# BUBLET/uav-airvision

Hardware: AMD Instinct MI355X
Metric: stereo frames/sec (LK+stereo+MSCKF-update) at 752x480 (higher is better)
Workload: dtype u8/int32 windows, f32 normal equations

## Files before the change

uav_airvision_amd/csrc/msckf.hip:

```cpp
#include <math.h>

#include <new>
#include <vector>

#include "av_common.h"

namespace {

constexpr int IMU_DIM = 21;

#ifndef AV_FILTER_WAVE_PRIO
#define AV_FILTER_WAVE_PRIO 3
#endif
#define AV_FILTER_PRIO() __builtin_amdgcn_s_setprio(AV_FILTER_WAVE_PRIO)

__device__ __forceinline__ double av_rsqrt_f64(double d)
{
    const bool tiny = d < 1e-280;
    const double ds = tiny ? d * 0x1p200 : d;
    double y = __builtin_amdgcn_rsq(ds);
    const double h = 0.5 * ds;
    y = y * (1.5 - h * y * y);
    y = y * (1.5 - h * y * y);
    return tiny ? y * 0x1p100 : y;
// ... 702 lines not shown
__global__ __attribute__((amdgpu_waves_per_eu(2, 3))) __launch_bounds__(256) void feature_kernel8(FeatArgs a) { feature_body<8>(a); }

static int msckf_lds_opt_in();

static int launch_feature_kernel(FeatArgs a, int cnt, int Mx, hipStream_t st)
{
    int rc0 = msckf_lds_opt_in();
    if (rc0) return rc0;
    a.Mmax = Mx; a.n_list = cnt;
    const int team = Mx <= 2 ? 16 : (Mx <= 4 ? 64 : 256);
    const size_t per = (feature_lds_bytes(Mx, team) + 7) / 8 * 8;
    a.team_doubles = (int)(per / 8);
    const size_t lds = per * (256 / team);
    if (lds > 160 * 1024) { av_set_error("MSCKF feature blocks: %d observations per feature need %zu B of LDS", Mx, lds); return AV_E_CAPACITY; }
    if (team == 16) hipLaunchKernelGGL(feature_kernel<16>, dim3((cnt + 15) / 16), dim3(256), lds, st, a);
    else if (team == 64) hipLaunchKernelGGL(feature_kernel<64>, dim3((cnt + 3) / 4), dim3(256), lds, st, a);
    else hipLaunchKernelGGL(feature_kernel<256>, dim3(cnt), dim3(256), lds, st, a);
    AV_LAUNCH_CHECK();
    return AV_OK;
}

struct PropArgs {
    double* P; int n, ld;
    double dt;
    double gyro[3], acc[3];
    double q_old[4];
    double q_new[4];
    double q_null[4], v_null[3], p_null[3];
    double v_new[3], p_new[3];
    double gravity[3];
    double noise[4];
};

constexpr int PROP_LDS_DOUBLES = 5 * IMU_DIM * IMU_DIM + IMU_DIM * 12;
template <bool EXT = false, int NT = 256>
__device__ __forceinline__ void propagate_body(const PropArgs& a, double* P11s = nullptr, double* PhiT = nullptr, double* ext = nullptr)
{
    __shared__ double own[EXT ? 1 : PROP_LDS_DOUBLES];
    double* const base = EXT ? ext : own;
    double* const F = base, * const F2 = F + IMU_DIM * IMU_DIM, * const Phi = F2 + IMU_DIM * IMU_DIM, * const T = Phi + IMU_DIM * IMU_DIM,
          * const Q = T + IMU_DIM * IMU_DIM, * const G = Q + IMU_DIM * IMU_DIM;
    __shared__ double Rwi[9], Rnull[9], Rnew[9], u[3], sv[3], w1[3], w2[3];
    const int tid = threadIdx.x;
    const int N = IMU_DIM;
    constexpr int Q1 = NT == 256 ? 64 : 1, Q2 = NT == 256 ? 128 : 2;
    constexpr int R1 = NT == 256 ? 64 : 9, R2 = NT == 256 ? 128 : 22, R3 = NT == 256 ? 192 : 43;
    for (int i = tid; i < N * N; i += NT) F[i] = 0.0;
    for (int i = tid; i < N * 12; i += NT) G[i] = 0.0;
    if (tid == 0 || tid == Q1 || tid == Q2) quat_to_rot(tid == 0 ? a.q_old : (tid == Q1 ? a.q_null : a.q_new), tid == 0 ? Rwi : (tid == Q1 ? Rnull : Rnew));
    __syncthreads();
    if (tid < 9) {
        const int r = tid / 3, c = tid - 3 * r;
        const double* w = a.gyro; const double* ac = a.acc;
        const double skw[9] = {0, -w[2], w[1], w[2], 0, -w[0], -w[1], w[0], 0};
        const double ska[9] = {0, -ac[2], ac[1], ac[2], 0, -ac[0], -ac[1], ac[0], 0};
        F[r * N + c] = -skw[r * 3 + c];
        F[r * N + 3 + c] = r == c ? -1.0 : 0.0;
        double s = 0;
        for (int k = 0; k < 3; ++k) s += Rwi[k * 3 + r] * ska[k * 3 + c];
        F[(6 + r) * N + c] = -s;
        F[(6 + r) * N + 9 + c] = -Rwi[c * 3 + r];
        F[(12 + r) * N + 6 + c] = r == c ? 1.0 : 0.0;
        G[r * 12 + c] = r == c ? -1.0 : 0.0;
        G[(3 + r) * 12 + 3 + c] = r == c ? 1.0 : 0.0;
        G[(6 + r) * 12 + 6 + c] = -Rwi[c * 3 + r];
        G[(9 + r) * 12 + 9 + c] = r == c ? 1.0 : 0.0;
    } else if (tid == R1) {
        for (int r = 0; r < 3; ++r) u[r] = Rnull[r * 3] * a.gravity[0] + Rnull[r * 3 + 1] * a.gravity[1] + Rnull[r * 3 + 2] * a.gravity[2];
        double uu = u[0] * u[0] + u[1] * u[1] + u[2] * u[2];
        for (int r = 0; r < 3; ++r) sv[r] = u[r] / uu;
    } else if (tid == R2) {
        double dv[3] = {a.v_null[0] - a.v_new[0], a.v_null[1] - a.v_new[1], a.v_null[2] - a.v_new[2]};
        double dp[3] = {a.dt * a.v_null[0] + a.p_null[0] - a.p_new[0], a.dt * a.v_null[1] + a.p_null[1] - a.p_new[1], a.dt * a.v_null[2] + a.p_null[2] - a.p_new[2]};
        const double* g = a.gravity;
        w1[0] = -dv[2] * g[1] + dv[1] * g[2]; w1[1] = dv[2] * g[0] - dv[0] * g[2]; w1[2] = -dv[1] * g[0] + dv[0] * g[1];
        w2[0] = -dp[2] * g[1] + dp[1] * g[2]; w2[1] = dp[2] * g[0] - dp[0] * g[2]; w2[2] = -dp[1] * g[0] + dp[0] * g[1];
    }
    __syncthreads();
    __shared__ unsigned frow[IMU_DIM], fcol[IMU_DIM], prow[IMU_DIM];
    for (int i = tid; i < N * N; i += NT) F[i] *= a.dt;
    if (tid >= R2 && tid < R2 + N) {
        const int r = tid - R2; unsigned m = 0;
        for (int k = 0; k < N; ++k) if (F[r * N + k] != 0.0) m |= 1u << k;
        frow[r] = m;
    } else if (tid >= R3 && tid < R3 + N) {
        const int c = tid - R3; unsigned m = 0;
        for (int k = 0; k < N; ++k) if (F[k * N + c] != 0.0) m |= 1u << k;
        fcol[c] = m;
    }
    __syncthreads();
    for (int i = tid; i < N * N; i += NT) {
        int r = i / N, c = i - r * N; double s = 0;
        for (unsigned m = frow[r]; m; m &= m - 1) { const int k = __builtin_ctz(m); s += F[r * N + k] * F[k * N + c]; }
        F2[i] = s;
    }
    __syncthreads();
    for (int i = tid; i < N * N; i += NT) {
        int r = i / N, c = i - r * N; double s = 0;
        for (unsigned m = fcol[c]; m; m &= m - 1) { const int k = __builtin_ctz(m); s += F2[r * N + k] * F[k * N + c]; }
        Phi[i] = (r == c ? 1.0 : 0.0) + F[i] + F2[i] / 2. + s / 6.;
    }
    __syncthreads();
    if (tid < 9) {
        int r = tid / 3, c = tid % 3; double s = 0;
        for (int k = 0; k < 3; ++k) s += Rnew[r * 3 + k] * Rnull[c * 3 + k];
        Phi[r * N + c] = s;
    } else if (tid >= R1 && tid < R1 + 6) {
        const int t6 = tid - R1, blk = t6 / 3, r = t6 % 3;
        const int row = (blk == 0 ? 6 : 12) + r;
        const double* wv = blk == 0 ? w1 : w2;
        const double p0 = Phi[row * N], p1 = Phi[row * N + 1], p2 = Phi[row * N + 2];
        const double Au = p0 * u[0] + p1 * u[1] + p2 * u[2];
        const double d = Au - wv[r];
        Phi[row * N] = p0 - d * sv[0]; Phi[row * N + 1] = p1 - d * sv[1]; Phi[row * N + 2] = p2 - d * sv[2];
    } else if (tid >= R2 && tid < R2 + N) {
        const int r = tid - R2; unsigned m = 0;
        for (int k = 0; k < N; ++k) if (Phi[r * N + k] != 0.0) m |= 1u << k;
        if (r < 3 || (r >= 6 && r < 9) || (r >= 12 && r < 15)) m |= 7u;
        prow[r] = m;
    }
    __syncthreads();
    for (int i = tid; i < N * 12; i += NT) {
        int r = i / 12, c = i - r * 12; double s = 0;
        for (unsigned m = prow[r]; m; m &= m - 1) { const int k = __builtin_ctz(m); s += Phi[r * N + k] * G[k * 12 + c]; }
        T[i] = s;
    }
    for (int i = tid; i < N * N; i += NT) {
        int r = i / N, c = i - r * N; double s = 0;
        if (P11s) { for (unsigned m = prow[r]; m; m &= m - 1) { const int k = __builtin_ctz(m); s += Phi[r * N + k] * P11s[k * N + c]; } }
        else      { for (unsigned m = prow[r]; m; m &= m - 1) { const int k = __builtin_ctz(m); s += Phi[r * N + k] * a.P[(size_t)k * a.ld + c]; } }
        F2[i] = s;
        if (P11s) {
            double s2 = 0;
            for (unsigned m = prow[r]; m; m &= m - 1) { const int k = __builtin_ctz(m); s2 += Phi[r * N + k] * PhiT[k * N + c]; }
            Q[i] = s2;
        }
    }
    __syncthreads();
    for (int i = tid; i < N * N; i += NT) {
        int r = i / N, c = i - r * N; double s = 0, q = 0;
        for (int k = 0; k < 12; ++k) q += T[r * 12 + k] * a.noise[k / 3] * T[c * 12 + k];
        q = q * a.dt;
        for (unsigned m = prow[c]; m; m &= m - 1) { const int k = __builtin_ctz(m); s += F2[r * N + k] * Phi[c * N + k]; }
        F[i] = s + q;
    }
    __syncthreads();
    if (P11s) {
        for (int i = tid; i < N * N; i += NT) {
            int r = i / N, c = i - r * N;
            PhiT[i] = Q[i];
            P11s[i] = (F[r * N + c] + F[c * N + r]) / 2.;
        }
        __syncthreads();
        return;
    }
    const int nc = a.n - N;
    for (int c0 = 0; c0 < nc; c0 += N) {
        const int w = min(N, nc - c0);
        for (int i = tid; i < N * w; i += NT) {
            int r = i / w, c = i - r * w; double s = 0;
            for (unsigned m = prow[r]; m; m &= m - 1) { const int k = __builtin_ctz(m); s += Phi[r * N + k] * a.P[(size_t)k * a.ld + N + c0 + c]; }
            T[i] = s;
        }
        __syncthreads();
        for (int i = tid; i < N * w; i += NT) {
            int r = i / w, c = i - r * w;
            a.P[(size_t)r * a.ld + N + c0 + c] = T[i];
            a.P[(size_t)(N + c0 + c) * a.ld + r] = T[i];
        }
        __syncthreads();
    }
    for (int i = tid; i < N * N; i += NT) {
        int r = i / N, c = i - r * N;
        a.P[(size_t)r * a.ld + c] = (F[r * N + c] + F[c * N + r]) / 2.;
    }
}

__global__ __launch_bounds__(256) void propagate_kernel(PropArgs a) { propagate_body(a); }
__global__ __launch_bounds__(256) void propagate_batch_kernel(const PropArgs* arr, const int* first)
{
    AV_FILTER_PRIO();
    __shared__ double P11s[IMU_DIM * IMU_DIM], PhiT[IMU_DIM * IMU_DIM];
    const int i0 = first[blockIdx.x], i1 = first[blockIdx.x + 1];
    if (i0 >= i1) return;
    const int tid = threadIdx.x, N = IMU_DIM;
    double* P = arr[i0].P; const int n = arr[i0].n, ld = arr[i0].ld;
    for (int i = tid; i < N * N; i += 256) { int r = i / N, c = i - r * N; P11s[i] = P[(size_t)r * ld + c]; PhiT[i] = r == c ? 1.0 : 0.0; }
    __syncthreads();
    for (int i = i0; i < i1; ++i) propagate_body(arr[i], P11s, PhiT);
    const int nc = n - N, tot = N * nc;
    constexpr int PER = (IMU_DIM * 6 * 31 + 255) / 256;
    double acc[PER];
#pragma unroll
    for (int u = 0; u < PER; ++u) {
        const int e = tid + 256 * u;
        double s = 0;
        if (e < tot) {
            const int r = e / nc, c = e - r * nc;
            for (int k = 0; k < N; ++k) s += PhiT[r * N + k] * P[(size_t)k * ld + N + c];
        }
        acc[u] = s;
// ... 1293 lines not shown
```

uav_airvision_amd/csrc/msckf_dev.inc:

```

namespace {

constexpr int DEV_BUCKETS = 2;
constexpr int DEV_IMU_BATCH = 16;
constexpr int DEV_LDS_KEYS = 2048;

enum { DFAIL_NONE = 0, DFAIL_CAMS = 1, DFAIL_FRAMES = 2, DFAIL_STACK = 3, DFAIL_PIVOT = 4, DFAIL_TABLE = 5, DFAIL_OBS = 6, DFAIL_ROWS = 7 };

struct DState {
    double ts;
    double q[4], p[3], v[3], bg[3], ba[3];
    double R_ic[9], t_ci[3];
    double qn[4], pn[3], vn[3];
    double gravity[3];
    double tracking_rate;
    long long next_imu_id;
    int n, ncam;
    int active;
    int failed;
    int first_img, null_aliased;
    int prune, rm0, rm1;
    int n_prune_steps;
    int n_two_pass;
    int resets;
};
struct DCtl {
    double t_frame;
    double q0[4], bg0[3], g0[3];
    int active, has_init, imu_first, imu_cnt;
};
struct DImu { double t, w[3], a[3]; };
struct DCov { int act, cnt, first, pad; AugArgs aa; };

struct DevArgs {
    int S, cap, FS, cs, max_cam, ld, rows_cap, obs_stride;
    unsigned long long* prof;
    int pool_rows;
    size_t pstride;
    double* P; double* scratch;
    DState* st; long long* cam_id; double* cam_q; double* cam_p; double* cam_qn; int* ncam; int* nstate; double* grav;
    int mcap, ns, hcells;
    long long* fr_id; double* fr_z; int* fr_fslot; int* fr_prev; int* fr_next; int* fr_n; int* pos_of; int* order; int* hdr; long long* births;
    long long* m_id; long long* m_birth; double* m_pos; int* m_init; int* m_nobs; int* m_tail; int* free_stack;
    int* hash_a; int* hash_b; int* hash_c; int* tmp_a; int* tmp_b; int* tmp_c; unsigned long long* keys; int* cand; int* e0; int* e1;
    int* f_off; int* obs_cam; double* obs_z; double* f_pos; int* f_dof; int* f_rowoff; int* f_valid; int* f_mslot; int* n_cand; int* over;
    int* t_off; int* t_obs_cam; double* t_obs_z;
    int* blist; int* tlist; int* cnt; int* cnt_next;
    const int* stacked; const double* dx;
    const DCtl* ctl; const DImu* imu; const long long* msg_ids; const double* msg_uv; const int* msg_n; int msg_cap;
    PropArgs* prop; DCov* cov;
    double* out;
    double R01[9], t01[3], noise[4], cov0[5];
    double trans_thr, pos_std_thr;
    double huber, precision, damping; int outer_max, inner_max;
    double* Hblk; double* rblk; size_t hstride, rstride; const double* chi2; double obs_noise; double* gamma; int* pass;
    const UpdArgs* updbase; UpdArgs* upd; int* cols; int cols_stride; int* blk_row; int* blk_len; int* stacked_out; double* work;
};

__device__ __forceinline__ TriArgs dev_tri_args(const DevArgs& a, bool prune)
{
    TriArgs t;
    t.n_feat = 0; t.obs_off = prune ? a.t_off : a.f_off; t.obs_cam = prune ? a.t_obs_cam : a.obs_cam; t.obs_z = prune ? a.t_obs_z : a.obs_z;
    t.cam_q = a.cam_q; t.cam_p = a.cam_p; t.feat_stream = nullptr; t.cam_stride = a.cs;
    for (int i = 0; i < 9; ++i) t.R01[i] = a.R01[i];
    for (int i = 0; i < 3; ++i) t.t01[i] = a.t01[i];
    t.huber = a.huber; t.precision = a.precision; t.damping = a.damping; t.outer_max = a.outer_max; t.inner_max = a.inner_max;
    t.out_pos = a.f_pos; t.out_valid = a.f_valid; t.list = nullptr; t.n_list_dev = nullptr; t.fs_stride = a.FS;
    t.f_mslot = prune ? a.f_mslot : nullptr; t.meta_pos = prune ? a.m_pos : nullptr; t.meta_init = prune ? a.m_init : nullptr; t.meta_stride = a.mcap;
    return t;
}
__device__ __forceinline__ void dev_triangulate_own(const DevArgs& a, const AvsStore& V, int s, int nc, bool prune)
{
    const TriArgs t = dev_tri_args(a, prune);
    const int wave = threadIdx.x >> 6, lane = threadIdx.x & 63;
    const size_t f0 = (size_t)s * a.FS;
    for (int k = wave; k < nc; k += (int)(blockDim.x >> 6)) if (V.tmp_b[k] >= 0) triangulate_one(t, (int)(f0 + k), lane);
    __syncthreads();
}

__device__ __forceinline__ AvsStore dev_store(const DevArgs& a, int s)
{
    AvsStore V;
    V.cap = a.cap; V.mcap = a.mcap; V.ns = a.ns; V.hcells = a.hcells;
// ... 111 lines not shown
            const int n = D->n, ld = a.ld;
            for (int k = 0; k < C.imu_cnt; ++k) {
                PropArgs pa;
                const DImu m = a.imu[C.imu_first + k];
                pa.P = P; pa.n = n; pa.ld = ld; pa.dt = m.t - D->ts;
                for (int i = 0; i < 3; ++i) { pa.gyro[i] = m.w[i] - D->bg[i]; pa.acc[i] = m.a[i] - D->ba[i]; pa.gravity[i] = D->gravity[i]; }
                for (int i = 0; i < 4; ++i) { pa.q_old[i] = D->q[i]; pa.noise[i] = a.noise[i]; }
                dev_predict_new_state(*D, pa.dt, pa.gyro, pa.acc);
                for (int i = 0; i < 4; ++i) { pa.q_new[i] = D->q[i]; pa.q_null[i] = D->qn[i]; }
                for (int i = 0; i < 3; ++i) { pa.v_null[i] = D->vn[i]; pa.p_null[i] = D->pn[i]; pa.v_new[i] = D->v[i]; pa.p_new[i] = D->p[i]; }
                for (int i = 0; i < 4; ++i) D->qn[i] = D->q[i];
                for (int i = 0; i < 3; ++i) { D->pn[i] = D->p[i]; D->vn[i] = D->v[i]; }
                D->null_aliased = 1;
                D->ts = m.t;
                a.prop[C.imu_first + k] = pa;
            }
            double Rwi[9], Rwc[9], tw[3], cq[4];
            h_to_rotation(D->q, Rwi);
            for (int r = 0; r < 3; ++r) for (int c = 0; c < 3; ++c) Rwc[r * 3 + c] = D->R_ic[r * 3] * Rwi[c] + D->R_ic[r * 3 + 1] * Rwi[3 + c] + D->R_ic[r * 3 + 2] * Rwi[6 + c];
            h_mtv(Rwi, D->t_ci, tw);
            h_to_quaternion(Rwc, cq);
            const size_t c = (size_t)s * a.cs + D->ncam;
            a.cam_id[c] = D->next_imu_id++;
            for (int i = 0; i < 4; ++i) { a.cam_q[4 * c + i] = cq[i]; a.cam_qn[4 * c + i] = cq[i]; }
            for (int i = 0; i < 3; ++i) a.cam_p[3 * c + i] = D->p[i] + tw[i];
            cv.act = 1; cv.cnt = C.imu_cnt;
            cv.aa.P = P; cv.aa.n = n; cv.aa.ld = ld;
            for (int i = 0; i < 9; ++i) cv.aa.R_ic[i] = D->R_ic[i];
            const double sk[9] = {0, -tw[2], tw[1], tw[2], 0, -tw[0], -tw[1], tw[0], 0};
            for (int i = 0; i < 9; ++i) cv.aa.sk[i] = sk[i];
            D->n = n + 6; D->ncam += 1;
            a.ncam[s] = D->ncam; a.nstate[s] = D->n;
            for (int i = 0; i < 3; ++i) a.grav[3 * s + i] = D->gravity[i];
        }
        a.cov[s] = cv;
        *Dg = L;
    }
}

template <int NT>
__global__ __launch_bounds__(NT) void dk_cov(DevArgs a)
{
    AV_FILTER_PRIO();
    __shared__ double P11s[IMU_DIM * IMU_DIM], PhiT[IMU_DIM * IMU_DIM], work[PROP_LDS_DOUBLES];
    const int s = blockIdx.x, tid = threadIdx.x, N = IMU_DIM;
    const DCov cv = a.cov[s];
    if (!cv.act) return;
    double* P = cv.aa.P;
    const int n = cv.aa.n, ld = cv.aa.ld;
    auto stamp = [&](int i) { if (a.prof && s == 0 && tid == 0) a.prof[i] = __builtin_amdgcn_s_memrealtime(); };
    stamp(0);
    if (cv.cnt > 0) {
        for (int i = tid; i < N * N; i += NT) { const int r = i / N, c = i - r * N; P11s[i] = P[(size_t)r * ld + c]; PhiT[i] = r == c ? 1.0 : 0.0; }
        __syncthreads();
        for (int k = 0; k < cv.cnt; ++k) propagate_body<true, NT>(a.prop[cv.first + k], P11s, PhiT, work);
        stamp(1);
        const int nc = n - N;
        constexpr int CW = 64, NRQ = NT / CW;
        const int cl = tid % CW, rq = tid / CW;
        for (int c0 = 0; c0 < nc; c0 += CW) {
            const int c = c0 + cl;
            const bool in = c < nc;
            __syncthreads();
            for (int k = rq; k < IMU_DIM; k += NRQ) work[k * CW + cl] = in ? P[(size_t)k * ld + N + c] : 0.0;
            __syncthreads();
#pragma unroll 1
            for (int r = rq; r < IMU_DIM; r += NRQ) {
                double sum = 0;
#pragma unroll 7
                for (int k = 0; k < IMU_DIM; ++k) sum += PhiT[r * N + k] * work[k * CW + cl];
                if (in) { P[(size_t)r * ld + N + c] = sum; P[(size_t)(N + c) * ld + r] = sum; }
            }
        }
        for (int i = tid; i < N * N; i += NT) { const int r = i / N, c = i - r * N; P[(size_t)r * ld + c] = P11s[i]; }
        __syncthreads();
    }
    stamp(2);
    augment_body<NT>(cv.aa);
}

__device__ void dev_build_candidates(const DevArgs& a, const AvsTeam& T, const AvsStore& V, int s, int nc, const int* cand, bool full,
                                     int i0, int i1, const int* e0, const int* e1, int ph, int* lb )
{
    const int tid = threadIdx.x;
    const size_t f0 = (size_t)s * a.FS, ob = (size_t)s * a.obs_stride;
    if (tid < 8) lb[tid] = 0;
    __syncthreads();
    int obs_run = 0, row_run = 0, tobs_run = 0;
    for (int base = 0; base < nc; base += (int)blockDim.x) {
        const int k = base + tid;
        const bool in = k < nc;
        const int fs = in ? cand[k] : 0;
        const int nall = in ? V.m_nobs[fs] : 0;
        const int nobs = full ? nall : (in ? 2 : 0);
        const int init = in ? V.m_init[fs] : 1;
        int to, tr, tt;
        const int o = obs_run + T.excl_scan(nobs, &to);
        const int r = row_run + T.excl_scan(in ? 4 * nobs - 3 : 0, &tr);
        const int t = tobs_run + T.excl_scan((!full && !init) ? nall : 0, &tt);
        if (in) {
            const size_t f = f0 + k;
            a.f_off[f] = (int)(ob + o); a.f_rowoff[f] = r; a.f_dof[f] = full ? nobs - 1 : 2; a.f_mslot[f] = fs;
            if (!full) a.t_off[f] = (int)(ob + t);
            if (full) (void)avs_collect(V, fs, a.obs_cam + ob + o, a.obs_z + 4 * (ob + o));
            else {
                a.obs_cam[ob + o] = i0; a.obs_cam[ob + o + 1] = i1;
                const double* z0 = V.fr_z + ((size_t)avs_lslot(e0[k]) * V.cap + avs_lidx(e0[k])) * 4;
// ... 209 lines not shown
            reset = m >= a.pos_std_thr;
        }
        s_reset = reset;
    }
    __syncthreads();
    if (s_reset) {
        AvsTeam T; T.red = red;
        const AvsStore V = dev_store(a, s);
        avs_clear(T, V);
        double* P = a.P + (size_t)s * a.pstride;
        for (int i = tid; i < IMU_DIM * IMU_DIM; i += (int)blockDim.x) {
            const int r = i / IMU_DIM, c = i - r * IMU_DIM;
            double v = 0.0;
            if (r == c) { const int blk[5] = {3, 6, 9, 15, 18}; for (int k = 0; k < 5; ++k) if (r >= blk[k] && r < blk[k] + 3) v = a.cov0[k]; }
            P[(size_t)r * a.ld + c] = v;
        }
        if (tid == 0) { D->ncam = 0; D->n = IMU_DIM; D->resets += 1; a.ncam[s] = 0; a.nstate[s] = IMU_DIM; }
    }
}
__global__ __launch_bounds__(256, 5) void dk_finish(DevArgs a)
{
    AV_FILTER_PRIO();
    dk_finish_body(a, blockIdx.x);
}


}

constexpr int DEV_RING = 3;
struct DevSlot {
    DCtl* ctl_h = nullptr; DCtl* ctl_d = nullptr;
    DImu* imu_h = nullptr; DImu* imu_d = nullptr; size_t imu_cap = 0;
    PropArgs* prop_d = nullptr;
    long long* ids_h = nullptr; double* uv_h = nullptr; int* n_h = nullptr;
    long long* ids_d = nullptr; double* uv_d = nullptr; int* n_d = nullptr;
    double* out_h = nullptr; int* cnt_h = nullptr;
    hipEvent_t done = nullptr;
    hipEvent_t t0[2] = {nullptr, nullptr}, t1[2] = {nullptr, nullptr}; bool t_used[2] = {false, false};
    bool in_flight = false;
};
struct DevPath {
    int cap = 0;
    DevArgs A;
    DevSlot slot[DEV_RING];
    double* out_d = nullptr; int* stacked0 = nullptr; int* stacked1 = nullptr; UpdArgs* updbase = nullptr; UpdArgs* upd = nullptr;
    DCov* cov_d = nullptr;
    int dk_wg = 0;
    int* cols = nullptr; int* blk_row = nullptr; int* blk_len = nullptr; int* clist = nullptr; int* again = nullptr;
    double* work = nullptr; double* gamma = nullptr; int* pass = nullptr;
    std::vector<void*> dev_allocs, host_allocs;
    int hint[16] = {0};
    bool have_hint = false;
    long long growths = 0, steps = 0;
};
```

uav_airvision_amd/csrc/msckf_dev_host.inc:

```
namespace {

constexpr int DEV_KCH = 136;

template <typename T>
int dev_alloc(DevPath* d, T** p, size_t count, int fill = 0)
{
    void* q = nullptr;
    AV_HIP(hipMalloc(&q, count * sizeof(T) + 256));
    AV_HIP(hipMemset(q, fill, count * sizeof(T) + 256));
    AV_HIP(hipStreamSynchronize(nullptr));
    d->dev_allocs.push_back(q);
    *p = reinterpret_cast<T*>(q);
    return AV_OK;
}
template <typename T>
int dev_pinned(DevPath* d, T** p, size_t count)
{
    void* q = nullptr;
    AV_HIP(hipHostMalloc(&q, count * sizeof(T) + 64, hipHostMallocDefault));
    memset(q, 0, count * sizeof(T) + 64);
    d->host_allocs.push_back(q);
    *p = reinterpret_cast<T*>(q);
    return AV_OK;
}

void dev_release(DevPath* d)
{
    if (!d) return;
    for (int k = 0; k < DEV_RING; ++k) {
        if (d->slot[k].done) (void)hipEventDestroy(d->slot[k].done);
        for (int ph = 0; ph < 2; ++ph) { if (d->slot[k].t0[ph]) (void)hipEventDestroy(d->slot[k].t0[ph]); if (d->slot[k].t1[ph]) (void)hipEventDestroy(d->slot[k].t1[ph]); }
    }
    for (void* p : d->dev_allocs) (void)hipFree(p);
    for (void* p : d->host_allocs) (void)hipHostFree(p);
    delete d;
}

__global__ __launch_bounds__(256) void dk_migrate(DevArgs o, DevArgs n)
{
    const int s = blockIdx.x, tid = threadIdx.x;
    const AvsStore A = dev_store(o, s), B = dev_store(n, s);
    for (int i = tid; i < A.ns; i += 256) { B.fr_n[i] = A.fr_n[i]; B.pos_of[i] = A.pos_of[i]; B.order[i] = A.order[i]; }
    for (int i = tid; i < AVS_HDR_WORDS; i += 256) B.hdr[i] = A.hdr[i];
    if (tid == 0) *B.births = *A.births;
    for (int sl = 0; sl < A.ns; ++sl) {
        const int cnt = A.fr_n[sl];
        for (int i = tid; i < cnt; i += 256) {
            const size_t a = (size_t)sl * A.cap + i, b = (size_t)sl * B.cap + i;
            B.fr_id[b] = A.fr_id[a]; B.fr_fslot[b] = A.fr_fslot[a]; B.fr_prev[b] = A.fr_prev[a]; B.fr_next[b] = A.fr_next[a];
            for (int e = 0; e < 4; ++e) B.fr_z[4 * b + e] = A.fr_z[4 * a + e];
        }
    }
    for (int i = tid; i < A.mcap; i += 256) {
        B.m_id[i] = A.m_id[i]; B.m_birth[i] = A.m_birth[i]; B.m_init[i] = A.m_init[i]; B.m_nobs[i] = A.m_nobs[i]; B.m_tail[i] = A.m_tail[i]; B.free_stack[i] = A.free_stack[i];
        for (int e = 0; e < 3; ++e) B.m_pos[(size_t)3 * i + e] = A.m_pos[(size_t)3 * i + e];
    }
}

int dev_reserve(av_msckf_batch* b, int cap)
{
    DevPath* d = b->dev;
    if (cap <= d->cap) return AV_OK;
    if (cap >= (1 << 24)) { av_set_error("batched MSCKF: message capacity %d exceeds the store's link format", cap); return AV_E_CAPACITY; }
    const bool grow = d->cap > 0;
// ... 2 lines not shown
    const size_t S = (size_t)b->S, cs = (size_t)b->cam_slots;
    DevArgs old = d->A;
    DevArgs& A = d->A;
    { const char* e = getenv("AV_DK_WG"); const int v = e ? atoi(e) : 0; d->dk_wg = (v == 256 || v == 64) ? v : 0; }
    A.S = b->S; A.cap = cap; A.FS = cap + 1; A.cs = b->cam_slots; A.max_cam = b->max_cam; A.ld = b->ld; A.rows_cap = b->rows_cap; A.pool_rows = (int)b_pool_rows(b, b->rows_cap);
    A.obs_stride = (int)((size_t)cap * cs); A.pstride = b->pstride; A.P = b->P; A.scratch = b->scratch;
    A.mcap = 2 * cap + 64; A.ns = b->cam_slots + 1;
    int hc = 64; while (hc < 2 * cap + 16) hc *= 2;
    A.hcells = hc;
    if ((size_t)S * A.FS >= (1u << 31) || S * (size_t)A.obs_stride >= (1u << 31)) { av_set_error("batched MSCKF: %zu streams x %d features exceed the 32-bit feature index", S, cap); return AV_E_CAPACITY; }
    const size_t nf = S * (size_t)A.FS + 8, no = S * (size_t)A.obs_stride + 8, ne = S * (size_t)A.ns * cap, nm = S * (size_t)A.mcap;
#define DA(ptr, cnt) if ((rc = dev_alloc(d, &(ptr), (size_t)(cnt)))) return rc;
#define DAF(ptr, cnt, fill) if ((rc = dev_alloc(d, &(ptr), (size_t)(cnt), fill))) return rc;
    if (!grow) {
        DA(A.st, S) DA(A.cam_id, S * cs) DA(A.cam_q, S * cs * 4) DA(A.cam_p, S * cs * 3) DA(A.cam_qn, S * cs * 4) DA(A.ncam, S) DA(A.nstate, S) DA(A.grav, S * 3)
        DA(A.n_cand, S) DA(A.over, S) DA(A.cnt, 32) DA(d->out_d, S * 12) DA(d->cov_d, S) DA(d->stacked0, S) DA(d->stacked1, S) DA(d->updbase, S) DA(d->upd, S * 2)
        DA(d->cols, S * 6 * cs) DA(d->clist, S + 8) DA(d->work, S * 8)
        DAF(A.pos_of, S * A.ns, 0xFF) DAF(A.order, S * A.ns, 0xFF) DA(A.fr_n, S * A.ns) DA(A.hdr, S * AVS_HDR_WORDS) DA(A.births, S)
    }
    DA(A.fr_id, ne) DA(A.fr_z, ne * 4) DA(A.fr_fslot, ne) DA(A.fr_prev, ne) DA(A.fr_next, ne)
    DA(A.m_id, nm) DA(A.m_birth, nm) DA(A.m_pos, nm * 3) DA(A.m_init, nm) DA(A.m_nobs, nm) DA(A.m_tail, nm) DA(A.free_stack, nm)
    DA(A.hash_a, S * hc) DA(A.hash_b, S * hc) DA(A.hash_c, S * hc)
    DA(A.tmp_a, S * cap) DA(A.tmp_b, S * cap) DA(A.tmp_c, S * cap) DA(A.keys, S * cap) DA(A.cand, S * cap) DA(A.e0, S * cap) DA(A.e1, S * cap)
    DA(A.f_off, nf) DA(A.obs_cam, no) DA(A.obs_z, no * 4) DA(A.f_pos, nf * 3) DA(A.f_dof, nf) DA(A.f_rowoff, nf) DA(A.f_valid, nf) DA(A.f_mslot, nf)
    DA(A.t_off, nf) DA(A.t_obs_cam, no) DA(A.t_obs_z, no * 4)
    DA(A.blist, 5 * S * cap + 8) DA(A.tlist, S * cap + 8) DA(d->blk_row, nf) DA(d->blk_len, nf) DA(d->again, nf) DA(d->gamma, nf) DA(d->pass, nf)
    for (int k = 0; k < DEV_RING; ++k) {
        DevSlot& sl = d->slot[k];
        if (!grow) {
            if ((rc = dev_pinned(d, &sl.ctl_h, S)) || (rc = dev_pinned(d, &sl.out_h, S * 12)) || (rc = dev_pinned(d, &sl.cnt_h, 16))) return rc;
            DA(sl.ctl_d, S) DA(sl.n_d, S)
            if ((rc = dev_pinned(d, &sl.n_h, S))) return rc;
            AV_HIP(hipEventCreateWithFlags(&sl.done, hipEventDisableTiming | hipEventBlockingSync));
            for (int ph = 0; ph < 2; ++ph) { AV_HIP(hipEventCreate(&sl.t0[ph])); AV_HIP(hipEventCreate(&sl.t1[ph])); }
        }
        DA(sl.ids_d, S * cap) DA(sl.uv_d, S * cap * 4)
        if ((rc = dev_pinned(d, &sl.ids_h, S * cap)) || (rc = dev_pinned(d, &sl.uv_h, S * cap * 4))) return rc;
    }
#undef DA
#undef DAF
    unpack_T01(b->T01, A.R01, A.t01);
    for (int i = 0; i < 4; ++i) A.noise[i] = b->noise[i];
    for (int i = 0; i < 5; ++i) A.cov0[i] = b->cov0[i];
    A.trans_thr = b->trans_thr; A.pos_std_thr = b->pos_std_thr;
    unpack_opt5(b->opt5, A);
    A.Hblk = b->Hblk; A.rblk = b->rblk; A.hstride = b->hstride; A.rstride = b->rstride; A.chi2 = b->chi2_dev; A.obs_noise = b->obs_noise;
    A.gamma = d->gamma; A.pass = d->pass; A.updbase = d->updbase; A.upd = d->upd; A.cols = d->cols; A.cols_stride = 6 * b->cam_slots;
    A.blk_row = d->blk_row; A.blk_len = d->blk_len; A.stacked_out = d->stacked1; A.work = d->work;
    A.stacked = nullptr; A.dx = b->dx; A.ctl = nullptr; A.imu = nullptr; A.prop = nullptr; A.cov = d->cov_d; A.msg_ids = nullptr; A.msg_uv = nullptr; A.msg_n = nullptr; A.msg_cap = cap; A.out = d->out_d;
    if (!grow) {
        std::vector<DState> st(S);
        for (size_t s = 0; s < S; ++s) {
            DState& D = st[s]; const BStream& T = b->st[s];
            memset(&D, 0, sizeof(D));
            D.q[3] = 1.0; D.qn[3] = 1.0; D.n = IMU_DIM; D.first_img = 1;
            for (int i = 0; i < 3; ++i) { D.v[i] = T.v[i]; D.t_ci[i] = T.t_ci[i]; D.gravity[i] = T.gravity[i]; }
            for (int i = 0; i < 9; ++i) D.R_ic[i] = T.R_ic[i];
        }
        AV_HIP(hipMemcpy(A.st, st.data(), sizeof(DState) * S, hipMemcpyHostToDevice));
        std::vector<int> n21(S, IMU_DIM);
        AV_HIP(hipMemcpy(A.nstate, n21.data(), sizeof(int) * S, hipMemcpyHostToDevice));
    } else {
        hipLaunchKernelGGL(dk_migrate, dim3((unsigned)S), dim3(256), 0, nullptr, old, A);
        AV_LAUNCH_CHECK();
        AV_HIP(hipDeviceSynchronize());
    }
    d->cap = cap;
    return AV_OK;
}

struct DevStamps {
    unsigned long long* dev = nullptr;
    int calls = 0;
    explicit DevStamps(bool on)
    {
        if (on && hipMalloc((void**)&dev, 256) == hipSuccess) { (void)hipMemset(dev, 0, 256); (void)hipStreamSynchronize(nullptr); } else dev = nullptr;
    }
    bool read(hipStream_t stm, unsigned long long t[32])
    {
        return dev && (++calls & 15) == 0 && hipStreamSynchronize(stm) == hipSuccess && hipMemcpy(t, dev, 256, hipMemcpyDeviceToHost) == hipSuccess;
    }
};
// ... 178 lines not shown
    return AV_OK;
}

int dev_enqueue(av_msckf_batch* b, int k, bool dev_msg, size_t n_imu, hipStream_t stm);

int dev_launch(av_msckf_batch* b, int k, const int64_t* ids, const double* uv, const int32_t* n_feat, int cap, const double* timestamps,
               bool dev_msg, hipEvent_t ready, hipStream_t stm)
{
    DevPath* d = b->dev;
    const int S = b->S;
    AV_HIP(hipSetDevice(b->device));
    int rc;
    if ((rc = sub_reserve(b, cap))) return rc;
    const bool first = d->cap == 0;
    const int rows_cap_before = d->A.rows_cap;
    if ((rc = dev_reserve(b, cap))) return rc;
    if (first || rows_cap_before != b->rows_cap) { if ((rc = dev_upload_updbase(b))) return rc; }
    DevSlot& sl = d->slot[k];
    if (sl.in_flight) { av_set_error("batched MSCKF: ring slot %d is still in flight", k); return AV_E_INVALID; }
    ++b->n_steps;
    if (b->debug_capture) for (BStream& T : b->st) for (int ph = 0; ph < 2; ++ph) { T.dbg_gamma[ph].clear(); T.dbg_dx[ph].clear(); T.dbg_P[ph].clear(); T.dbg_rows[ph] = 0; T.dbg_n[ph] = 0; }
    size_t n_imu = 0;
    for (int s = 0; s < S; ++s) {
        BStream& T = b->st[s];
        std::lock_guard<std::mutex> g(T.mu);
        T.active = !T.failed && T.gravity_set && timestamps[s] >= 0 && T.gravity_time <= timestamps[s];
        if (!T.active) continue;
        const double t0 = T.first_img ? timestamps[s] : T.ts;
        for (const BImu& m : T.imu) { if (m.t < t0) continue; if (m.t > timestamps[s]) break; ++n_imu; }
    }
    if (n_imu > sl.imu_cap) {
        const size_t ncap = n_imu + n_imu / 2 + (size_t)S * 16 + 64;
        if (sl.imu_cap) { AV_HIP(hipStreamSynchronize(stm)); ++d->growths; }
        if ((rc = dev_pinned(d, &sl.imu_h, ncap)) || (rc = dev_alloc(d, &sl.imu_d, ncap)) || (rc = dev_alloc(d, &sl.prop_d, ncap))) return rc;
        sl.imu_cap = ncap;
    }
    size_t w = 0;
    for (int s = 0; s < S; ++s) {
        BStream& T = b->st[s];
        DCtl& C = sl.ctl_h[s];
        C.t_frame = timestamps[s]; C.active = T.active ? 1 : 0; C.has_init = 0; C.imu_first = (int)w; C.imu_cnt = 0;
        if (!T.active) continue;
        std::lock_guard<std::mutex> g(T.mu);
        if (!T.dev_init_sent) {
            T.dev_init_sent = true; C.has_init = 1;
            for (int i = 0; i < 4; ++i) C.q0[i] = T.q[i];
            for (int i = 0; i < 3; ++i) { C.bg0[i] = T.bg[i]; C.g0[i] = T.gravity[i]; }
        }
        if (T.first_img) { T.first_img = false; T.ts = timestamps[s]; }
        size_t used = 0;
        for (const BImu& m : T.imu) {
            if (m.t < T.ts) { ++used; continue; }
            if (m.t > timestamps[s] || w >= sl.imu_cap) break;
            DImu& o = sl.imu_h[w++];
            o.t = m.t;
            for (int i = 0; i < 3; ++i) { o.w[i] = m.w[i]; o.a[i] = m.a[i]; }
            ++C.imu_cnt; ++used;
            T.ts = m.t;
        }
        T.imu.erase(T.imu.begin(), T.imu.begin() + used);
    }
    if (!dev_msg) {
        for (int s = 0; s < S; ++s) {
            const int nk = n_feat[s] < 0 ? 0 : (n_feat[s] > cap ? cap : n_feat[s]);
            sl.n_h[s] = nk;
            memcpy(sl.ids_h + (size_t)s * d->cap, ids + (size_t)s * cap, sizeof(long long) * nk);
            memcpy(sl.uv_h + (size_t)s * d->cap * 4, uv + (size_t)s * cap * 4, sizeof(double) * 4 * nk);
        }
    }
    if (dev_msg && ready) AV_HIP(hipStreamWaitEvent(stm, ready, 0));
    if ((rc = dev_enqueue(b, k, dev_msg, w, stm))) { (void)hipMemsetAsync(d->A.cnt, 0, sizeof(int) * 32, stm); return rc; }
    ++d->steps;
    AV_HIP(hipEventRecord(sl.done, stm));
    sl.in_flight = true;
    return AV_OK;
}

int dev_enqueue(av_msckf_batch* b, int k, bool dev_msg, size_t n_imu, hipStream_t stm)
{
    DevPath* d = b->dev;
    DevSlot& sl = d->slot[k];
    const int S = b->S;
    int rc;
    AV_HIP(hipMemcpyAsync(sl.ctl_d, sl.ctl_h, sizeof(DCtl) * S, hipMemcpyHostToDevice, stm));
    if (n_imu) AV_HIP(hipMemcpyAsync(sl.imu_d, sl.imu_h, sizeof(DImu) * n_imu, hipMemcpyHostToDevice, stm));
    if (!dev_msg) {
        AV_HIP(hipMemcpyAsync(sl.n_d, sl.n_h, sizeof(int) * S, hipMemcpyHostToDevice, stm));
        AV_HIP(hipMemcpyAsync(sl.ids_d, sl.ids_h, sizeof(long long) * S * d->cap, hipMemcpyHostToDevice, stm));
        AV_HIP(hipMemcpyAsync(sl.uv_d, sl.uv_h, sizeof(double) * 4 * S * d->cap, hipMemcpyHostToDevice, stm));
    }
    DevArgs a = d->A;
    a.ctl = sl.ctl_d; a.imu = sl.imu_d; a.prop = sl.prop_d; a.msg_ids = sl.ids_d; a.msg_uv = sl.uv_d; a.msg_n = sl.n_d; a.msg_cap = d->cap;
    const int par = (int)((d->steps + 1) & 1);
    a.cnt = d->A.cnt + 16 * par; a.cnt_next = d->A.cnt + 16 * (par ^ 1);
    a.prof = dev_uprof().dev ? dev_uprof().dev + 16 : nullptr;
    const int dk_wg = d->dk_wg ? d->dk_wg : (S >= 1024 ? 64 : 256);
    hipLaunchKernelGGL(dk_state, dim3((S + 63) / 64), dim3(64), 0, stm, a);
    hipLaunchKernelGGL(dk_begin4, dim3(S), dim3(dk_wg), 0, stm, a);
    if (dk_wg == 64) hipLaunchKernelGGL(dk_cov<64>, dim3(S), dim3(64), 0, stm, a);
    else hipLaunchKernelGGL(dk_cov<256>, dim3(S), dim3(256), 0, stm, a);
    AV_LAUNCH_CHECK();
    if ((rc = dev_phase(b, 0, stm, sl, a.cnt))) return rc;
    if (b->debug_capture && (rc = dev_debug_capture(b, 0, stm))) return rc;
    a.stacked = d->stacked0;
    hipLaunchKernelGGL(dk_mid, dim3(S), dim3(dk_wg), 0, stm, a);
    AV_LAUNCH_CHECK();
    if ((rc = dev_phase(b, 1, stm, sl, a.cnt))) return rc;
    if (b->debug_capture && (rc = dev_debug_capture(b, 1, stm))) return rc;
    a.stacked = d->stacked1;
    hipLaunchKernelGGL(dk_finish, dim3(S), dim3(dk_wg), 0, stm, a);
    AV_LAUNCH_CHECK();
    AV_HIP(hipMemcpyAsync(sl.out_h, d->out_d, sizeof(double) * 12 * S, hipMemcpyDeviceToHost, stm));
    AV_HIP(hipMemcpyAsync(sl.cnt_h, a.cnt, sizeof(int) * 16, hipMemcpyDeviceToHost, stm));
    return AV_OK;
}

int dev_finish(av_msckf_batch* b, int k, double* out)
{
    DevPath* d = b->dev;
    DevSlot& sl = d->slot[k];
    if (!sl.in_flight) return AV_OK;
    AV_HIP(hipEventSynchronize(sl.done));
    sl.in_flight = false;
    memcpy(out, sl.out_h, sizeof(double) * 12 * b->S);
    for (int i = 0; i < 16; ++i) d->hint[i] = sl.cnt_h[i];
    d->have_hint = true;
    for (int ph = 0; ph < 2; ++ph) if (sl.t_used[ph]) {
        float ms = 0;
        if (hipEventElapsedTime(&ms, sl.t0[ph], sl.t1[ph]) == hipSuccess) b->w_chain_ms += ms; else ++b->w_chain_dropped;
        sl.t_used[ph] = false;
    }
    return AV_OK;
}

const char* dev_fail_message(int code, int* av_code)
{
    *av_code = code == DFAIL_PIVOT ? AV_E_NUMERIC : AV_E_CAPACITY;
    switch (code) {
    case DFAIL_CAMS: return "stream exceeds the camera-state slots of its window";
    case DFAIL_FRAMES: return "more frames in the stream's window than the observation store holds (or a message wider than its capacity)";
    case DFAIL_STACK: return "stream stacks more blocks in one update than the back end holds (4096 blocks / the compression stage's row maps)";
    case DFAIL_PIVOT: return "a Cholesky factorisation of the stacked update met a non-positive or non-finite pivot (rank-deficient Gram matrix or corrupt covariance); update skipped, stream stopped";
    case DFAIL_TABLE: return "the stream's feature table is full";
    case DFAIL_ROWS: return "the lost features of one frame need more rows than the stream's block buffers and the shared overflow pool hold (AV_MSCKF_POOL_ROWS)";
    default: return "stream stopped";
    }
}

int dev_read_state(av_msckf_batch* b, int s, DState* D)
{
    AV_HIP(hipSetDevice(b->device));
    AV_HIP(hipMemcpy(D, b->dev->A.st + s, sizeof(DState), hipMemcpyDeviceToHost));
    return AV_OK;
}

}
```

Before: 200,500.

## Precompute IMU transition matrices in parallel kernel before serial covariance chain

Splits IMU propagation into a new dk_phi kernel that builds Phi, the process-noise matrix and row masks for every IMU sample in its own workgroup, one per sample. The serial per-stream dk_cov loop then only applies the precomputed Phi/Q to the covariance and prefetches the next record into registers. This takes the F/F2/Phi/T construction off the sequential dependency chain, at the cost of an extra kernel launch and a global-memory round trip for the PhiRec buffers. Inactive streams mark their samples with n=0 so dk_phi skips them.

```diff
diff --git a/uav_airvision_amd/csrc/msckf.hip b/uav_airvision_amd/csrc/msckf.hip
--- a/uav_airvision_amd/csrc/msckf.hip
+++ b/uav_airvision_amd/csrc/msckf.hip
@@ -758,14 +758,21 @@
     double noise[4];
 };
 
-constexpr int PROP_LDS_DOUBLES = 5 * IMU_DIM * IMU_DIM + IMU_DIM * 12;
-template <bool EXT = false, int NT = 256>
-__device__ __forceinline__ void propagate_body(const PropArgs& a, double* P11s = nullptr, double* PhiT = nullptr, double* ext = nullptr)
-{
-    __shared__ double own[EXT ? 1 : PROP_LDS_DOUBLES];
-    double* const base = EXT ? ext : own;
+struct PhiRec {
+    double Phi[IMU_DIM * IMU_DIM];
+    double Q[IMU_DIM * IMU_DIM];
+    double dt;
+    unsigned prow[IMU_DIM];
+    int pad;
+};
+
+constexpr int PROP_PHI_DOUBLES = 3 * IMU_DIM * IMU_DIM + 2 * IMU_DIM * 12;
+constexpr int PROP_LDS_DOUBLES = PROP_PHI_DOUBLES + IMU_DIM * IMU_DIM;
+template <int NT>
+__device__ __forceinline__ void propagate_phi(const PropArgs& a, double* base, unsigned* prow)
+{
     double* const F = base, * const F2 = F + IMU_DIM * IMU_DIM, * const Phi = F2 + IMU_DIM * IMU_DIM, * const T = Phi + IMU_DIM * IMU_DIM,
-          * const Q = T + IMU_DIM * IMU_DIM, * const G = Q + IMU_DIM * IMU_DIM;
+          * const G = T + IMU_DIM * 12;
     __shared__ double Rwi[9], Rnull[9], Rnew[9], u[3], sv[3], w1[3], w2[3];
     const int tid = threadIdx.x;
     const int N = IMU_DIM;
@@ -803,7 +810,7 @@
         w2[0] = -dp[2] * g[1] + dp[1] * g[2]; w2[1] = dp[2] * g[0] - dp[0] * g[2]; w2[2] = -dp[1] * g[0] + dp[0] * g[1];
     }
     __syncthreads();
-    __shared__ unsigned frow[IMU_DIM], fcol[IMU_DIM], prow[IMU_DIM];
+    __shared__ unsigned frow[IMU_DIM], fcol[IMU_DIM];
     for (int i = tid; i < N * N; i += NT) F[i] *= a.dt;
     if (tid >= R2 && tid < R2 + N) {
         const int r = tid - R2; unsigned m = 0;
@@ -851,48 +858,87 @@
         for (unsigned m = prow[r]; m; m &= m - 1) { const int k = __builtin_ctz(m); s += Phi[r * N + k] * G[k * 12 + c]; }
         T[i] = s;
     }
-    for (int i = tid; i < N * N; i += NT) {
-        int r = i / N, c = i - r * N; double s = 0;
-        if (P11s) { for (unsigned m = prow[r]; m; m &= m - 1) { const int k = __builtin_ctz(m); s += Phi[r * N + k] * P11s[k * N + c]; } }
-        else      { for (unsigned m = prow[r]; m; m &= m - 1) { const int k = __builtin_ctz(m); s += Phi[r * N + k] * a.P[(size_t)k * a.ld + c]; } }
-        F2[i] = s;
-        if (P11s) {
-            double s2 = 0;
-            for (unsigned m = prow[r]; m; m &= m - 1) { const int k = __builtin_ctz(m); s2 += Phi[r * N + k] * PhiT[k * N + c]; }
-            Q[i] = s2;
-        }
-    }
-    __syncthreads();
-    for (int i = tid; i < N * N; i += NT) {
-        int r = i / N, c = i - r * N; double s = 0, q = 0;
-        for (int k = 0; k < 12; ++k) q += T[r * 12 + k] * a.noise[k / 3] * T[c * 12 + k];
-        q = q * a.dt;
-        for (unsigned m = prow[c]; m; m &= m - 1) { const int k = __builtin_ctz(m); s += F2[r * N + k] * Phi[c * N + k]; }
-        F[i] = s + q;
-    }
-    __syncthreads();
-    if (P11s) {
-        for (int i = tid; i < N * N; i += NT) {
-            int r = i / N, c = i - r * N;
-            PhiT[i] = Q[i];
-            P11s[i] = (F[r * N + c] + F[c * N + r]) / 2.;
+    __syncthreads();
+}
+__device__ __forceinline__ double propagate_noise(const PropArgs& a, const double* T, int r, int c)
+{
+    double q = 0;
+    for (int k = 0; k < 12; ++k) q += T[r * 12 + k] * a.noise[k / 3] * T[c * 12 + k];
+    return q;
+}
+template <int NT, bool BATCH, class QF>
+__device__ __forceinline__ void propagate_cov(const double* Phi, const unsigned* prow, double dt, double* F2, double* Fb,
+                                              double* P11s, double* PhiT, const double* Pg, int ld, QF qf)
+{
+    constexpr int N = IMU_DIM, PER = (N * N + NT - 1) / NT;
+    const int tid = threadIdx.x;
+    double pt[PER];
+#pragma unroll
+    for (int u = 0; u < PER; ++u) {
+        const int i = tid + NT * u;
+        if (i < N * N) {
+            int r = i / N, c = i - r * N; double s = 0;
+            if (BATCH) { for (unsigned m = prow[r]; m; m &= m - 1) { const int k = __builtin_ctz(m); s += Phi[r * N + k] * P11s[k * N + c]; } }
+            else       { for (unsigned m = prow[r]; m; m &= m - 1) { const int k = __builtin_ctz(m); s += Phi[r * N + k] * Pg[(size_t)k * ld + c]; } }
+            F2[i] = s;
+            if (BATCH) {
+                double s2 = 0;
+                for (unsigned m = prow[r]; m; m &= m - 1) { const int k = __builtin_ctz(m); s2 += Phi[r * N + k] * PhiT[k * N + c]; }
+                pt[u] = s2;
+            }
+        }
+    }
+    __syncthreads();
+#pragma unroll
+    for (int u = 0; u < PER; ++u) {
+        const int i = tid + NT * u;
+        if (i < N * N) {
+            int r = i / N, c = i - r * N; double s = 0;
+            if (BATCH) PhiT[i] = pt[u];
+            for (unsigned m = prow[c]; m; m &= m - 1) { const int k = __builtin_ctz(m); s += F2[r * N + k] * Phi[c * N + k]; }
+            Fb[i] = __builtin_fma(qf(u, r, c), dt, s);
+        }
+    }
+    __syncthreads();
+    if (BATCH) {
+#pragma unroll
+        for (int u = 0; u < PER; ++u) {
+            const int i = tid + NT * u;
+            if (i < N * N) {
+                int r = i / N, c = i - r * N;
+                P11s[i] = (Fb[r * N + c] + Fb[c * N + r]) / 2.;
+            }
         }
         __syncthreads();
-        return;
-    }
+    }
+}
+
+__device__ __forceinline__ void propagate_body(const PropArgs& a, double* P11s = nullptr, double* PhiT = nullptr)
+{
+    constexpr int NT = 256;
+    __shared__ double own[PROP_LDS_DOUBLES];
+    __shared__ unsigned prow[IMU_DIM];
+    double* const F = own, * const F2 = F + IMU_DIM * IMU_DIM, * const Phi = F2 + IMU_DIM * IMU_DIM, * const T = Phi + IMU_DIM * IMU_DIM,
+          * const Q = own + PROP_PHI_DOUBLES;
+    const int tid = threadIdx.x;
+    const int N = IMU_DIM;
+    propagate_phi<NT>(a, own, prow);
+    auto qf = [&](int, int r, int c) { return propagate_noise(a, T, r, c); };
+    if (P11s) { propagate_cov<NT, true>(Phi, prow, a.dt, F2, F, P11s, PhiT, nullptr, 0, qf); return; }
+    propagate_cov<NT, false>(Phi, prow, a.dt, F2, F, nullptr, nullptr, a.P, a.ld, qf);
     const int nc = a.n - N;
     for (int c0 = 0; c0 < nc; c0 += N) {
         const int w = min(N, nc - c0);
         for (int i = tid; i < N * w; i += NT) {
             int r = i / w, c = i - r * w; double s = 0;
             for (unsigned m = prow[r]; m; m &= m - 1) { const int k = __builtin_ctz(m); s += Phi[r * N + k] * a.P[(size_t)k * a.ld + N + c0 + c]; }
-            T[i] = s;
+            Q[i] = s;
         }
         __syncthreads();
         for (int i = tid; i < N * w; i += NT) {
             int r = i / w, c = i - r * w;
-            a.P[(size_t)r * a.ld + N + c0 + c] = T[i];
-            a.P[(size_t)(N + c0 + c) * a.ld + r] = T[i];
+            a.P[(size_t)r * a.ld + N + c0 + c] = Q[i];
+            a.P[(size_t)(N + c0 + c) * a.ld + r] = Q[i];
         }
         __syncthreads();
     }
diff --git a/uav_airvision_amd/csrc/msckf_dev.inc b/uav_airvision_amd/csrc/msckf_dev.inc
--- a/uav_airvision_amd/csrc/msckf_dev.inc
+++ b/uav_airvision_amd/csrc/msckf_dev.inc
@@ -49,6 +49,7 @@
     const int* stacked; const double* dx;
     const DCtl* ctl; const DImu* imu; const long long* msg_ids; const double* msg_uv; const int* msg_n; int msg_cap;
     PropArgs* prop; DCov* cov;
+    PhiRec* phi;
     double* out;
     double R01[9], t01[3], noise[4], cov0[5];
     double trans_thr, pos_std_thr;
@@ -226,31 +227,76 @@
             D->n = n + 6; D->ncam += 1;
             a.ncam[s] = D->ncam; a.nstate[s] = D->n;
             for (int i = 0; i < 3; ++i) a.grav[3 * s + i] = D->gravity[i];
+        } else {
+            for (int k = 0; k < C.imu_cnt; ++k) a.prop[C.imu_first + k].n = 0;
         }
         a.cov[s] = cv;
         *Dg = L;
     }
 }
 
+__global__ __launch_bounds__(64) void dk_phi(DevArgs a)
+{
+    AV_FILTER_PRIO();
+    __shared__ double work[PROP_PHI_DOUBLES];
+    __shared__ unsigned prow[IMU_DIM];
+    constexpr int N = IMU_DIM;
+    const int tid = threadIdx.x;
+    const PropArgs& pa = a.prop[blockIdx.x];
+    if (pa.n == 0) return;
+    propagate_phi<64>(pa, work, prow);
+    const double* Phi = work + 2 * N * N, * T = Phi + N * N;
+    PhiRec& R = a.phi[blockIdx.x];
+    for (int i = tid; i < N * N; i += 64) {
+        const int r = i / N, c = i - r * N;
+        R.Phi[i] = Phi[i];
+        R.Q[i] = propagate_noise(pa, T, r, c);
+    }
+    if (tid < N) R.prow[tid] = prow[tid];
+    if (tid == 0) R.dt = pa.dt;
+}
+
 template <int NT>
 __global__ __launch_bounds__(NT) void dk_cov(DevArgs a)
 {
     AV_FILTER_PRIO();
-    __shared__ double P11s[IMU_DIM * IMU_DIM], PhiT[IMU_DIM * IMU_DIM], work[PROP_LDS_DOUBLES];
-    const int s = blockIdx.x, tid = threadIdx.x, N = IMU_DIM;
-    const DCov cv = a.cov[s];
+    constexpr int N = IMU_DIM, NN = N * N, PER = (NN + NT - 1) / NT, CW = 64;
+    __shared__ double lds[5 * NN];
+    __shared__ unsigned prow[N];
+    static_assert(4 * NN >= N * CW, "the cross block's panel lives in the IMU block and the work matrices");
+    double* const PhiT = lds, * const P11s = PhiT + NN, * const Phi = P11s + NN, * const F2 = Phi + NN, * const Fb = F2 + NN, * const work = P11s;
+    const int s = blockIdx.x, tid = threadIdx.x;
+    const DCov& cv = a.cov[s];
     if (!cv.act) return;
     double* P = cv.aa.P;
-    const int n = cv.aa.n, ld = cv.aa.ld;
+    const int n = cv.aa.n, ld = cv.aa.ld, cnt = cv.cnt;
     auto stamp = [&](int i) { if (a.prof && s == 0 && tid == 0) a.prof[i] = __builtin_amdgcn_s_memrealtime(); };
     stamp(0);
-    if (cv.cnt > 0) {
-        for (int i = tid; i < N * N; i += NT) { const int r = i / N, c = i - r * N; P11s[i] = P[(size_t)r * ld + c]; PhiT[i] = r == c ? 1.0 : 0.0; }
-        __syncthreads();
-        for (int k = 0; k < cv.cnt; ++k) propagate_body<true, NT>(a.prop[cv.first + k], P11s, PhiT, work);
+    if (cnt > 0) {
+        const PhiRec* rec = a.phi + cv.first;
+        double nPhi[PER], nQ[PER], Qr[PER], ndt;
+        unsigned nrow = 0;
+        auto fetch = [&](const PhiRec& R) {
+#pragma unroll
+            for (int u = 0; u < PER; ++u) { const int i = tid + NT * u; nPhi[u] = i < NN ? R.Phi[i] : 0.0; nQ[u] = i < NN ? R.Q[i] : 0.0; }
+            if (tid < N) nrow = R.prow[tid];
+            ndt = R.dt;
+        };
+        fetch(rec[0]);
+        for (int i = tid; i < NN; i += NT) { const int r = i / N, c = i - r * N; P11s[i] = P[(size_t)r * ld + c]; PhiT[i] = r == c ? 1.0 : 0.0; }
+        for (int k = 0; k < cnt; ++k) {
+#pragma unroll
+            for (int u = 0; u < PER; ++u) { const int i = tid + NT * u; if (i < NN) Phi[i] = nPhi[u]; Qr[u] = nQ[u]; }
+            if (tid < N) prow[tid] = nrow;
+            const double dt = ndt;
+            __syncthreads();
+            if (k + 1 < cnt) fetch(rec[k + 1]);
+            propagate_cov<NT, true>(Phi, prow, dt, F2, Fb, P11s, PhiT, nullptr, 0, [&](int u, int, int) { return Qr[u]; });
+        }
         stamp(1);
+        for (int i = tid; i < N * N; i += NT) { const int r = i / N, c = i - r * N; P[(size_t)r * ld + c] = P11s[i]; }
         const int nc = n - N;
-        constexpr int CW = 64, NRQ = NT / CW;
+        constexpr int NRQ = NT / CW;
         const int cl = tid % CW, rq = tid / CW;
         for (int c0 = 0; c0 < nc; c0 += CW) {
             const int c = c0 + cl;
@@ -266,7 +312,6 @@
                 if (in) { P[(size_t)r * ld + N + c] = sum; P[(size_t)(N + c) * ld + r] = sum; }
             }
         }
-        for (int i = tid; i < N * N; i += NT) { const int r = i / N, c = i - r * N; P[(size_t)r * ld + c] = P11s[i]; }
         __syncthreads();
     }
     stamp(2);
@@ -542,11 +587,12 @@
     DCtl* ctl_h = nullptr; DCtl* ctl_d = nullptr;
     DImu* imu_h = nullptr; DImu* imu_d = nullptr; size_t imu_cap = 0;
     PropArgs* prop_d = nullptr;
+    PhiRec* phi_d = nullptr;
     long long* ids_h = nullptr; double* uv_h = nullptr; int* n_h = nullptr;
     long long* ids_d = nullptr; double* uv_d = nullptr; int* n_d = nullptr;
     double* out_h = nullptr; int* cnt_h = nullptr;
     hipEvent_t done = nullptr;
-    hipEvent_t t0[2] = {nullptr, nullptr}, t1[2] = {nullptr, nullptr}; bool t_used[2] = {false, false};
+    hipEvent_t t0[3] = {nullptr, nullptr, nullptr}, t1[3] = {nullptr, nullptr, nullptr}; bool t_used[3] = {false, false, false};
     bool in_flight = false;
 };
 struct DevPath {
diff --git a/uav_airvision_amd/csrc/msckf_dev_host.inc b/uav_airvision_amd/csrc/msckf_dev_host.inc
--- a/uav_airvision_amd/csrc/msckf_dev_host.inc
+++ b/uav_airvision_amd/csrc/msckf_dev_host.inc
@@ -29,7 +29,7 @@
     if (!d) return;
     for (int k = 0; k < DEV_RING; ++k) {
         if (d->slot[k].done) (void)hipEventDestroy(d->slot[k].done);
-        for (int ph = 0; ph < 2; ++ph) { if (d->slot[k].t0[ph]) (void)hipEventDestroy(d->slot[k].t0[ph]); if (d->slot[k].t1[ph]) (void)hipEventDestroy(d->slot[k].t1[ph]); }
+        for (int ph = 0; ph < 3; ++ph) { if (d->slot[k].t0[ph]) (void)hipEventDestroy(d->slot[k].t0[ph]); if (d->slot[k].t1[ph]) (void)hipEventDestroy(d->slot[k].t1[ph]); }
     }
     for (void* p : d->dev_allocs) (void)hipFree(p);
     for (void* p : d->host_allocs) (void)hipHostFree(p);
@@ -98,7 +98,7 @@
             DA(sl.ctl_d, S) DA(sl.n_d, S)
             if ((rc = dev_pinned(d, &sl.n_h, S))) return rc;
             AV_HIP(hipEventCreateWithFlags(&sl.done, hipEventDisableTiming | hipEventBlockingSync));
-            for (int ph = 0; ph < 2; ++ph) { AV_HIP(hipEventCreate(&sl.t0[ph])); AV_HIP(hipEventCreate(&sl.t1[ph])); }
+            for (int ph = 0; ph < 3; ++ph) { AV_HIP(hipEventCreate(&sl.t0[ph])); AV_HIP(hipEventCreate(&sl.t1[ph])); }
         }
         DA(sl.ids_d, S * cap) DA(sl.uv_d, S * cap * 4)
         if ((rc = dev_pinned(d, &sl.ids_h, S * cap)) || (rc = dev_pinned(d, &sl.uv_h, S * cap * 4))) return rc;
@@ -113,7 +113,7 @@
     A.Hblk = b->Hblk; A.rblk = b->rblk; A.hstride = b->hstride; A.rstride = b->rstride; A.chi2 = b->chi2_dev; A.obs_noise = b->obs_noise;
     A.gamma = d->gamma; A.pass = d->pass; A.updbase = d->updbase; A.upd = d->upd; A.cols = d->cols; A.cols_stride = 6 * b->cam_slots;
     A.blk_row = d->blk_row; A.blk_len = d->blk_len; A.stacked_out = d->stacked1; A.work = d->work;
-    A.stacked = nullptr; A.dx = b->dx; A.ctl = nullptr; A.imu = nullptr; A.prop = nullptr; A.cov = d->cov_d; A.msg_ids = nullptr; A.msg_uv = nullptr; A.msg_n = nullptr; A.msg_cap = cap; A.out = d->out_d;
+    A.stacked = nullptr; A.dx = b->dx; A.ctl = nullptr; A.imu = nullptr; A.prop = nullptr; A.phi = nullptr; A.cov = d->cov_d; A.msg_ids = nullptr; A.msg_uv = nullptr; A.msg_n = nullptr; A.msg_cap = cap; A.out = d->out_d;
     if (!grow) {
         std::vector<DState> st(S);
         for (size_t s = 0; s < S; ++s) {
@@ -358,7 +358,8 @@
     if (n_imu > sl.imu_cap) {
         const size_t ncap = n_imu + n_imu / 2 + (size_t)S * 16 + 64;
         if (sl.imu_cap) { AV_HIP(hipStreamSynchronize(stm)); ++d->growths; }
-        if ((rc = dev_pinned(d, &sl.imu_h, ncap)) || (rc = dev_alloc(d, &sl.imu_d, ncap)) || (rc = dev_alloc(d, &sl.prop_d, ncap))) return rc;
+        if ((rc = dev_pinned(d, &sl.imu_h, ncap)) || (rc = dev_alloc(d, &sl.imu_d, ncap)) || (rc = dev_alloc(d, &sl.prop_d, ncap)) ||
+            (rc = dev_alloc(d, &sl.phi_d, ncap))) return rc;
         sl.imu_cap = ncap;
     }
     size_t w = 0;
@@ -416,13 +417,18 @@
         AV_HIP(hipMemcpyAsync(sl.uv_d, sl.uv_h, sizeof(double) * 4 * S * d->cap, hipMemcpyHostToDevice, stm));
     }
     DevArgs a = d->A;
-    a.ctl = sl.ctl_d; a.imu = sl.imu_d; a.prop = sl.prop_d; a.msg_ids = sl.ids_d; a.msg_uv = sl.uv_d; a.msg_n = sl.n_d; a.msg_cap = d->cap;
+    a.ctl = sl.ctl_d; a.imu = sl.imu_d; a.prop = sl.prop_d; a.phi = sl.phi_d; a.msg_ids = sl.ids_d; a.msg_uv = sl.uv_d; a.msg_n = sl.n_d; a.msg_cap = d->cap;
     const int par = (int)((d->steps + 1) & 1);
     a.cnt = d->A.cnt + 16 * par; a.cnt_next = d->A.cnt + 16 * (par ^ 1);
     a.prof = dev_uprof().dev ? dev_uprof().dev + 16 : nullptr;
     const int dk_wg = d->dk_wg ? d->dk_wg : (S >= 1024 ? 64 : 256);
     hipLaunchKernelGGL(dk_state, dim3((S + 63) / 64), dim3(64), 0, stm, a);
     hipLaunchKernelGGL(dk_begin4, dim3(S), dim3(dk_wg), 0, stm, a);
+    if (n_imu) {
+        if (b->work_timing) { AV_HIP(hipEventRecord(sl.t0[2], stm)); sl.t_used[2] = true; }
+        hipLaunchKernelGGL(dk_phi, dim3((unsigned)n_imu), dim3(64), 0, stm, a);
+        if (sl.t_used[2]) AV_HIP(hipEventRecord(sl.t1[2], stm));
+    }
     if (dk_wg == 64) hipLaunchKernelGGL(dk_cov<64>, dim3(S), dim3(64), 0, stm, a);
     else hipLaunchKernelGGL(dk_cov<256>, dim3(S), dim3(256), 0, stm, a);
     AV_LAUNCH_CHECK();
@@ -451,7 +457,7 @@
     memcpy(out, sl.out_h, sizeof(double) * 12 * b->S);
     for (int i = 0; i < 16; ++i) d->hint[i] = sl.cnt_h[i];
     d->have_hint = true;
-    for (int ph = 0; ph < 2; ++ph) if (sl.t_used[ph]) {
+    for (int ph = 0; ph < 3; ++ph) if (sl.t_used[ph]) {
         float ms = 0;
         if (hipEventElapsedTime(&ms, sl.t0[ph], sl.t1[ph]) == hipSuccess) b->w_chain_ms += ms; else ++b->w_chain_dropped;
         sl.t_used[ph] = false;
```

New measurement: 198,600. No clear change (-1.0%).
